# skyplane-project/skyplane

Measured on NVIDIA H100. Metric: chunk-pipeline GB/s (raw input), higher is better.
Workload: dtype u8/u32

## Files before the change

skyplane_b200/csrc/lz4.cuh:

```cuda
#pragma once
#include <stdint.h>

namespace sky {

constexpr uint32_t kBlock = 65536;
#ifndef SKY_LZ4_ENTRIES
#define SKY_LZ4_ENTRIES 4096
#endif
constexpr uint32_t kEntries = SKY_LZ4_ENTRIES;
constexpr uint32_t kTableBytes = kEntries * 4;
constexpr uint32_t kMinMatch = 4;
constexpr uint32_t kMfLimit = 12;
constexpr uint32_t kLastLiterals = 5;
constexpr unsigned kFull = 0xffffffffu;

__device__ __forceinline__ void warp_copy(uint8_t *dst, const uint8_t *src, uint32_t n, unsigned lane) {
    if (n < 64) {
        for (uint32_t base = 0; base < n; base += 32) {
            const uint32_t k = base + lane;
            uint8_t b = 0;
            if (k < n) b = src[k];
            __syncwarp();
            if (k < n) dst[k] = b;
        }
// ... 181 lines not shown
__device__ __forceinline__ void sts16(uint32_t a, uint32_t v) { asm volatile("st.shared.u16 [%0], %1;" ::"r"(a), "h"((uint16_t)v) : "memory"); }

__device__ __forceinline__ void mbar_init(uint64_t *bar, uint32_t count) {
    asm volatile("mbarrier.init.shared::cta.b64 [%0], %1;" ::"r"(smem_u32(bar)), "r"(count) : "memory");
}
__device__ __forceinline__ void mbar_arrive(uint64_t *bar) {
    asm volatile("mbarrier.arrive.shared::cta.b64 _, [%0];" ::"r"(smem_u32(bar)) : "memory");
}
__device__ __forceinline__ void mbar_arrive_expect_tx(uint64_t *bar, uint32_t bytes) {
    asm volatile("mbarrier.arrive.expect_tx.shared::cta.b64 _, [%0], %1;" ::"r"(smem_u32(bar)), "r"(bytes) : "memory");
}
__device__ __forceinline__ bool mbar_try_wait(uint64_t *bar, uint32_t parity) {
    uint32_t ok;
    asm volatile("{\n\t.reg .pred p;\n\tmbarrier.try_wait.parity.shared::cta.b64 p, [%1], %2;\n\tselp.u32 %0, 1, 0, p;\n\t}"
                 : "=r"(ok) : "r"(smem_u32(bar)), "r"(parity) : "memory");
    return ok != 0;
}
__device__ __forceinline__ bool mbar_try_wait_hint(uint64_t *bar, uint32_t parity, uint32_t ns) {
    uint32_t ok;
    asm volatile("{\n\t.reg .pred p;\n\tmbarrier.try_wait.parity.shared::cta.b64 p, [%1], %2, %3;\n\tselp.u32 %0, 1, 0, p;\n\t}"
                 : "=r"(ok) : "r"(smem_u32(bar)), "r"(parity), "r"(ns) : "memory");
    return ok != 0;
}
__device__ __forceinline__ void mbar_wait(uint64_t *bar, uint32_t parity) {
    while (!mbar_try_wait_hint(bar, parity, 20000u)) {}
}
__device__ __forceinline__ void bulk_load(void *smem_dst, const void *gsrc, uint32_t bytes, uint64_t *bar) {
    asm volatile("cp.async.bulk.shared::cluster.global.mbarrier::complete_tx::bytes [%0], [%1], %2, [%3];"
                 ::"r"(smem_u32(smem_dst)), "l"(gsrc), "r"(bytes), "r"(smem_u32(bar)) : "memory");
}

__device__ __forceinline__ uint32_t div255(uint32_t x) { return (x * 0x8081u) >> 23; }
__device__ __forceinline__ uint32_t seq_bytes_fast(uint32_t ll, uint32_t ml) {
    uint32_t s = 1 + ll + (ll >= 15 ? div255(ll - 15) + 1 : 0);
    if (ml) s += 2 + (ml >= 19 ? div255(ml - 19) + 1 : 0);
    return s;
}
__device__ __forceinline__ uint32_t load32s(uint32_t in_s, uint32_t pos) {
    const uint32_t a = in_s + (pos & ~3u);
    return __funnelshift_r(lds32(a), lds32(a + 4), (pos & 3u) * 8u);
}

template <class Load4>
__device__ __forceinline__ uint32_t extend_coop(Load4 load4, uint32_t mpos, uint32_t mcand, uint32_t mlen, uint32_t maxlen, unsigned lane) {
    for (;;) {
        const uint32_t o = mlen + lane * 4;
        uint32_t cnt = 0;
        if (o < maxlen) {
            const uint32_t x = load4(mpos + o) ^ load4(mcand + o);
            cnt = x ? (uint32_t)(__ffs(x) - 1) >> 3 : 4u;
            cnt = min(cnt, maxlen - o);
        }
        const unsigned fullm = __ballot_sync(kFull, cnt == 4);
        if (fullm == kFull) {
            mlen += 128;
            continue;
        }
        const int f = __ffs(~fullm) - 1;
        return mlen + 4 * f + __shfl_sync(kFull, cnt, f);
    }
}
__device__ __forceinline__ uint32_t extend_coop_s(uint32_t in32, uint32_t mpos, uint32_t mcand, uint32_t mlen, uint32_t maxlen,
                                                  unsigned lane) {
    return extend_coop([in32](uint32_t pos) { return load32s(in32, pos); }, mpos, mcand, mlen, maxlen, lane);
}

__device__ __noinline__ uint32_t flush_seqs(uint8_t *__restrict__ out, uint32_t op, const uint8_t *in, uint32_t q0, uint32_t q1,
                                            uint32_t nseq, bool skip_first, unsigned lane) {
    const uint32_t in32 = smem_u32(in);
    const bool act = lane < nseq && !(skip_first && lane == 0);
    const uint32_t ll = q0 & 0xffffu, ml = q0 >> 16, lit = q1 & 0xffffu, off = q1 >> 16;
    const uint32_t mcode = ml - kMinMatch;
    const uint32_t nl = ll >= 15 ? div255(ll - 15) + 1 : 0, nm = mcode >= 15 ? div255(mcode - 15) + 1 : 0;
    const uint32_t sz = act ? 3 + ll + nl + nm : 0;
    uint32_t incl = sz;
#pragma unroll
    for (int d = 1; d < 32; d <<= 1) {
        const uint32_t t = __shfl_up_sync(kFull, incl, d);
        if ((int)lane >= d) incl += t;
    }
    const uint32_t total = __shfl_sync(kFull, incl, 31);
    uint32_t lit_o = 0;
    if (act) {
        uint32_t o = op + incl - sz;
        out[o++] = (uint8_t)(((ll < 15 ? ll : 15) << 4) | (mcode < 15 ? mcode : 15));
        if (nl) {
            for (uint32_t k = 0; k + 1 < nl; k++) out[o + k] = 255;
            out[o + nl - 1] = (uint8_t)(ll - 15 - (nl - 1) * 255);
            o += nl;
        }
        lit_o = o;
        if (ll < kCoopLit) {
            uint32_t k = 0;
            for (; k + 4 <= ll; k += 4) {
                const uint32_t w = load32s(in32, lit + k);
                out[o + k] = (uint8_t)w;
                out[o + k + 1] = (uint8_t)(w >> 8);
                out[o + k + 2] = (uint8_t)(w >> 16);
                out[o + k + 3] = (uint8_t)(w >> 24);
            }
            const uint32_t rem = ll - k;
            if (rem) {
                const uint32_t w = load32s(in32, lit + k);
                out[o + k] = (uint8_t)w;
                if (rem > 1) out[o + k + 1] = (uint8_t)(w >> 8);
                if (rem > 2) out[o + k + 2] = (uint8_t)(w >> 16);
            }
        }
        o += ll;
        out[o] = (uint8_t)off;
        out[o + 1] = (uint8_t)(off >> 8);
        o += 2;
        if (nm) {
            for (uint32_t k = 0; k + 1 < nm; k++) out[o + k] = 255;
            out[o + nm - 1] = (uint8_t)(mcode - 15 - (nm - 1) * 255);
        }
    }
    __syncwarp();
    unsigned big = __ballot_sync(kFull, act && ll >= kCoopLit);
    while (big) {
        const int l = __ffs(big) - 1;
        big &= big - 1;
        warp_copy(out + __shfl_sync(kFull, lit_o, l), in + __shfl_sync(kFull, lit, l), __shfl_sync(kFull, ll, l), lane);
    }
    return op + total;
}

__device__ __forceinline__ uint32_t bfind(uint32_t x) {
    uint32_t r;
    asm("bfind.u32 %0, %1;" : "=r"(r) : "r"(x));
    return r;
}
__device__ __forceinline__ void near_slot(uint32_t &n, uint32_t hf, uint32_t c3, uint32_t c4, uint32_t c8) {
    asm volatile(
        "{\n\t"
        ".reg .pred p, q;\n\t"
        ".reg .b32 t;\n\t"
        "shfl.sync.up.b32 t|p, %1, 8, 0, 0xffffffff;\n\t"
        "setp.eq.and.u32 q, t, %1, p;\n\t"
        "selp.u32 %0, %4, %0, q;\n\t"
        "shfl.sync.up.b32 t|p, %1, 4, 0, 0xffffffff;\n\t"
        "setp.eq.and.u32 q, t, %1, p;\n\t"
        "selp.u32 %0, %3, %0, q;\n\t"
        "shfl.sync.up.b32 t|p, %1, 3, 0, 0xffffffff;\n\t"
        "setp.eq.and.u32 q, t, %1, p;\n\t"
        "selp.u32 %0, %2, %0, q;\n\t"
        "}"
        : "+r"(n)
        : "r"(hf), "r"(c3), "r"(c4), "r"(c8));
}
__device__ __forceinline__ void red_max_s(uint32_t a, uint32_t v) {
    asm volatile("red.shared.max.u32 [%0], %1;" ::"r"(a), "r"(v) : "memory");
}
template <class Turn>
__device__ __forceinline__ uint32_t probe_batch(uint32_t in_s, uint32_t tab_s, uint32_t offs_s, uint32_t masks_s, uint32_t seg_pos,
                                                uint32_t slog, uint32_t batch, uint32_t mflimit, unsigned lane, Turn turn) {
    const uint32_t pstep = 32u << slog;
    uint32_t p = seg_pos + ((batch * 256u + lane) << slog);
    const uint32_t selv = 0x3210u + 0x1111u * (p & 3u), selb = 0x4440u | (p & 3u);
    const uint32_t offs_l = offs_s + (batch * 256u + lane) * 2u;
    const uint32_t c3 = 0x30000u << slog, c4 = 0x40000u << slog, c8 = 0x80000u << slog;
    uint32_t idx[8], mine[8], e[8], near[8], anyhit = 0;
#pragma unroll
    for (int k = 0; k < 8; k++) {
        const uint32_t pc = min(p, mflimit);
        const uint32_t a = in_s + (pc & ~3u);
        const uint32_t w0 = lds32(a), w1 = lds32(a + 4);
        uint32_t hf = __byte_perm(w0, w1, selv) * 2654435761u;
        hf = __byte_perm(w1, 0u, selb) * 0x85EBCA6Bu + hf;
        idx[k] = __umulhi(hf, kEntries) * 4u;
        mine[k] = __byte_perm(p, hf, 0x1065);
        near[k] = 0u;
        near_slot(near[k], hf, c3, c4, c8);
        p += pstep;
    }
    turn();
#pragma unroll
    for (int k = 0; k < 8; k++) {
        e[k] = lds32(tab_s + idx[k]);
        __syncwarp();
        red_max_s(tab_s + idx[k], mine[k]);
        __syncwarp();
    }
#pragma unroll
    for (int k = 0; k < 8; k++) {
        uint32_t d = mine[k] - e[k];
        if (near[k]) d = near[k];
        const uint32_t off = d >> 16;
        const unsigned hits = __ballot_sync(kFull, (d & 0xffffu) == 0u && off != 0u);
        anyhit |= hits;
        if (lane == 0) sts32(masks_s + (batch * 8u + (uint32_t)k) * 4u, hits);
        sts16(offs_l + (uint32_t)k * 64u, off);
    }
    return anyhit;
}

__device__ __forceinline__ SegRec parse_segment(const uint8_t *in, const SegSlot *slot, uint8_t *__restrict__ scr, uint32_t L,
                                                unsigned lane) {
    const uint32_t in32 = smem_u32(in), offs_s = smem_u32(slot->offs);
    const uint32_t seg_pos = slot->seg_pos, slog = slot->slog;
    const uint32_t mflimit = L - kMfLimit, matchlimit = L - kLastLiterals;
    const uint32_t n_real = ((mflimit - seg_pos) >> slog) + 1u;
    const uint32_t mymask = slot->masks[lane] & ~__funnelshift_lc(0u, 0xffffffffu, min(max(n_real, lane * 32u) - lane * 32u, 32u));
    const uint32_t seg_lim = seg_pos + (kSegSlots << slog);
    const uint32_t mlim = min(matchlimit, seg_lim);
    const uint32_t seg_end = seg_lim > mflimit ? L : seg_lim;
    const uint32_t round_up = (1u << slog) - 1u;
    const uint32_t dl = lane < 23 ? lane : lane - 32u;
    const uint32_t jrel = lane < 23 ? lane : 31u - lane;
    const bool fwd_lane = lane < 23;
    uint32_t anchor = seg_pos, cur = seg_pos, nseq = 0, q0 = 0, q1 = 0, mbytes = 0;
    uint32_t first_q0 = 0, first_q1 = 0;
    bool first_pending = true;
    unsigned nz = __ballot_sync(kFull, mymask != 0u);
    uint32_t m = 0, gbase = 0, sbase = 0;
    for (;;) {
        if (m == 0) {
            if (nz == 0) break;
            const int g = __ffs(nz) - 1;
            nz &= nz - 1;
            m = __shfl_sync(kFull, mymask, g);
            sbase = (uint32_t)g * 32u;
            gbase = seg_pos + (sbase << slog);
            m &= __funnelshift_lc(0u, 0xffffffffu, (max(cur, gbase) - gbase + round_up) >> slog);
            if (m == 0) continue;
        }
        const uint32_t bit = bfind(m & (0u - m));
        uint32_t pos = gbase + (bit << slog);
        const uint32_t off = lds16(offs_s + (sbase + bit) * 2u);
        const uint32_t cand = pos - off;
        const uint32_t maxlen = mlim - pos;
        const uint32_t room = min(min(pos - anchor, cand), 8u);
        bool ok = false;
        if (jrel < (fwd_lane ? maxlen : room)) ok = lds8(in32 + pos + dl) == lds8(in32 + cand + dl);
        const unsigned z = ~__ballot_sync(kFull, ok) | 0x00800000u;
        uint32_t mlen = bfind(z & (0u - z));
        if (mlen - kMinMatch >= 23u - kMinMatch) {
            if (mlen < kMinMatch) {
                m &= m - 1;
                continue;
            }
            if (maxlen > 23u) mlen = extend_coop_s(in32, pos, cand, 23u, maxlen, lane);
        }
        const uint32_t back = (uint32_t)__clz(z);
        const uint32_t end = pos + mlen;
        pos -= back;
        mlen += back;
        const uint32_t r0 = (pos - anchor) | (mlen << 16), r1 = anchor | (off << 16);
        if (lane == nseq) {
            q0 = r0;
            q1 = r1;
        }
        anchor = cur = end;
        m &= __funnelshift_lc(0u, 0xffffffffu, (cur - gbase + round_up) >> slog);
        if (++nseq == 32) {
            if (first_pending) {
                first_q0 = __shfl_sync(kFull, q0, 0);
                first_q1 = __shfl_sync(kFull, q1, 0);
            }
            mbytes = flush_seqs(scr, mbytes, in, q0, q1, 32, first_pending, lane);
            first_pending = false;
            nseq = 0;
        }
    }
    if (nseq) {
        if (first_pending) {
            first_q0 = __shfl_sync(kFull, q0, 0);
            first_q1 = __shfl_sync(kFull, q1, 0);
        }
        mbytes = flush_seqs(scr, mbytes, in, q0, q1, nseq, first_pending, lane);
    }
    SegRec r;
    r.seg_pos = seg_pos;
    r.lead_ml = first_q0;
    r.off_t = (first_q1 >> 16) | ((seg_end - anchor) << 16);
    r.mbytes = mbytes;
    return r;
}

}
```

skyplane_b200/csrc/skychunk.cu:

```cuda

#include <cuda_runtime.h>
#include <stdint.h>
#include <stdio.h>
#include <string.h>

#include <algorithm>
#include <memory>
#include <new>
#include <numeric>
#include <string>
#include <utility>
#include <vector>

#include "../../include/skychunk.h"
#include "frame.cuh"
#include "lz4.cuh"
#include "lz4dec.cuh"
#include "lz4hc.cuh"
#include "lz4verify.cuh"
#include "md5.cuh"
#include "secretbox.cuh"

namespace sky {

#ifndef SKY_PARSERS
#define SKY_PARSERS 12
#endif
constexpr int kParsers = SKY_PARSERS;
constexpr int kProbers = 2;
constexpr int kWarps = kProbers + kParsers;
constexpr int kThreads = kWarps * 32;
#ifndef SKY_RING_EXTRA
#define SKY_RING_EXTRA 2
#endif
constexpr int kRing = kParsers + SKY_RING_EXTRA;
constexpr int kMd5WarpsPerCta = 4;
constexpr uint32_t kRingBytes = SKY_MD5_SLOTS * 2048;
constexpr int kCtasPerSm = 2;
constexpr uint64_t kMaxChunkBlocks = 1ull << 21;

struct Ctl {
    uint64_t in_full;
    uint64_t full[kRing], empty[kRing];
    BlockDesc desc[2];
    uint32_t claim;
    volatile uint32_t block_end_seq;
    volatile uint32_t nseg;
    volatile uint32_t seg_hit[4];
    uint32_t raw, last_lits, tail_off;
    uint64_t data;
    uint32_t size;
    PendingChecksum pend;
};
constexpr uint32_t kInOff = 0;
constexpr uint32_t kTabOff = kInOff + kInBytes;
constexpr uint32_t kRingOff = kTabOff + kTableBytes;
constexpr uint32_t kRecOff = kRingOff + kRing * (uint32_t)sizeof(SegSlot);
constexpr uint32_t kPlanOff = kRecOff + kMaxSegs * (uint32_t)sizeof(SegRec);
constexpr uint32_t kCtlOff = kPlanOff + kMaxSegs * (uint32_t)sizeof(SegPlan);
constexpr uint32_t kSmemBytes = (kCtlOff + (uint32_t)sizeof(Ctl) + 127u) & ~127u;
static_assert(kSmemBytes <= 232448 / 2 - 1024, "two CTAs per SM need <= 112.5 KiB each: lower SKY_PARSERS or SKY_LZ4_ENTRIES");
static_assert(kEntries % 128 == 0, "SKY_LZ4_ENTRIES must be a multiple of 128");
static_assert(kMd5WarpsPerCta * kRingBytes <= kInBytes, "the MD5 rings live in the block buffer of a digest CTA");
static_assert(sizeof(SegSlot) % 16 == 0 && sizeof(SegRec) == 16 && sizeof(SegPlan) == 16, "layout");

template <int kId>
__device__ __forceinline__ void bar_arrive() { asm volatile("bar.arrive %0, 64;" ::"n"(kId) : "memory"); }
template <int kId>
__device__ __forceinline__ void bar_wait() { asm volatile("bar.sync %0, 64;" ::"n"(kId) : "memory"); }

template <bool kXxh, bool kBlkChk>
__device__ __forceinline__ void fused_body(const Params &p) {
    extern __shared__ __align__(128) uint8_t smem[];
    const unsigned warp = threadIdx.x >> 5, lane = threadIdx.x & 31;
    uint8_t *in = smem + kInOff;
    uint32_t *tab = reinterpret_cast<uint32_t *>(smem + kTabOff);
    SegSlot *ring = reinterpret_cast<SegSlot *>(smem + kRingOff);
    SegRec *recs = reinterpret_cast<SegRec *>(smem + kRecOff);
    SegPlan *plans = reinterpret_cast<SegPlan *>(smem + kPlanOff);
    Ctl *ctl = reinterpret_cast<Ctl *>(smem + kCtlOff);
    uint32_t smem_s = smem_u32(smem);
    asm volatile("" : "+r"(smem_s));

    const bool do_md5 = (p.flags & SKY_F_MD5) != 0, do_lz4 = (p.flags & SKY_F_LZ4) != 0;
    if (warp == 0 && lane == 0) {
        mbar_init(&ctl->in_full, 1);
        for (int i = 0; i < kRing; i++) {
            mbar_init(&ctl->full[i], 1);
            mbar_init(&ctl->empty[i], 1);
        }
        ctl->claim = 0;
        if constexpr (kBlkChk) ctl->pend.data = nullptr;
        asm volatile("fence.mbarrier_init.release.cluster;" ::: "memory");
    }
    __syncthreads();

    if (do_md5 && blockIdx.x < p.n_md5_ctas) {
        if (warp < kMd5WarpsPerCta) {
            for (uint32_t g = warp * p.n_md5_ctas + blockIdx.x; g < p.n_groups; g += p.n_md5_ctas * kMd5WarpsPerCta) {
                const uint32_t c = p.md5_order[g * 32 + lane];
                const bool active = c != 0xffffffffu;
                const uint8_t *src = nullptr;
                uint64_t len = 0;
                if (active) {
                    src = p.chunks[c].src;
                    len = p.chunks[c].len;
                }
                const uint32_t x = md5_warp<kXxh>(reinterpret_cast<uint32_t *>(in + warp * kRingBytes), src, len, active,
                                                  p.md5_out + (size_t)(active ? c : 0) * 16, lane);
                if constexpr (kXxh) {
                    if (active) p.xxh_out[c] = x;
                }
                __syncwarp();
            }
        }
        if (!do_lz4) return;
        __syncthreads();
    }
    if (!do_lz4) return;

    uint8_t *scratch = p.scratch + (size_t)blockIdx.x * kScratchBytes;
    uint32_t gseq = 0;
    uint32_t batches_done = 0;
    uint32_t my_seq = 0;
    bool have_claim = false;
    uint32_t in_phase = 0;
    constexpr unsigned kSumWarp = kWarps - 1;
    for (uint32_t it = 0;; it++) {
        BlockDesc *dsc = &ctl->desc[it & 1];
        if (warp == 0 && lane == 0) {
            claim_block(p, dsc);
            ctl->block_end_seq = 0xffffffffu;
            ctl->nseg = 0;
        }
        __syncthreads();
        if (!dsc->valid) {
            if constexpr (kBlkChk) {
                if (warp == kSumWarp) run_pending(&ctl->pend, lane);
            }
            break;
        }
        const uint8_t *src = dsc->src;
        const uint32_t L = dsc->L;

        if (warp < kProbers) {
            if (warp == 0) {
                if (lane == 0) load_block(in, src, L, &ctl->in_full);
                uint4 *t4 = reinterpret_cast<uint4 *>(tab);
                const uint4 z = make_uint4(0, 0, 0, 0);
#pragma unroll 4
                for (uint32_t k = lane; k < kEntries / 4; k += 32) t4[k] = z;
                __syncwarp();
            }
            mbar_wait(&ctl->in_full, in_phase);
            in_phase ^= 1;
            uint32_t nseg = 0;
            if (L >= kMfLimit + 1) {
                const uint32_t mflimit = L - kMfLimit;
                uint32_t seg_pos = 0, slog = 0;
                while (seg_pos <= mflimit) {
                    if (nseg >= 2) {
                        const bool h = ctl->seg_hit[(nseg - 2) & 3u] != 0u;
                        slog = h ? 0u : min(slog + 1u, kMaxStepLog);
                    }
                    const uint32_t si = gseq % kRing, ph = (gseq / kRing) & 1u;
                    SegSlot *slot = ring + si;
#pragma unroll 1
                    for (uint32_t b = warp; b < 4; b += kProbers) {
                        const uint32_t slot_s = smem_s + kRingOff + si * (uint32_t)sizeof(SegSlot);
                        const uint32_t hits = probe_batch(smem_s + kInOff, smem_s + kTabOff, slot_s + (uint32_t)offsetof(SegSlot, offs),
                                                          slot_s + (uint32_t)offsetof(SegSlot, masks), seg_pos, slog, b, mflimit, lane, [&]() {
                            if (warp == 0) {
                                if (batches_done) bar_wait<2>();
                                if (b == 0) mbar_wait(&ctl->empty[si], ph ^ 1u);
                            } else {
                                bar_wait<1>();
                            }
                        });
                        batches_done = 1;
                        if (lane == 0) {
                            ctl->seg_hit[nseg & 3u] = (b == 0 ? 0u : ctl->seg_hit[nseg & 3u]) | hits;
                            if (b == 0) {
                                slot->seg_pos = seg_pos;
                                slot->slog = slog;
                                slot->sidx = nseg;
                            }
                        }
                        __syncwarp();
                        if (b == 3 && lane == 0) mbar_arrive(&ctl->full[si]);
                        __threadfence_block();
                        if (warp == 0) bar_arrive<1>(); else bar_arrive<2>();
                    }
                    seg_pos += kSegSlots << slog;
                    gseq++;
                    nseg++;
                }
            }
            if (warp == kProbers - 1 && lane == 0) {
                ctl->nseg = nseg;
                __threadfence_block();
                atomicExch(const_cast<uint32_t *>(&ctl->block_end_seq), gseq);
            }
        } else {
            mbar_wait(&ctl->in_full, in_phase);
            in_phase ^= 1;
            for (;;) {
                if (!have_claim) {
                    uint32_t t = 0;
                    if (lane == 0) t = atomicAdd(&ctl->claim, 1u);
                    my_seq = __shfl_sync(kFull, t, 0);
                    have_claim = true;
                }
                const uint32_t si = my_seq % kRing, ph = (my_seq / kRing) & 1u;
                bool got = true;
                while (!mbar_try_wait_hint(&ctl->full[si], ph, 1000u)) {
                    if (atomicAdd(const_cast<uint32_t *>(&ctl->block_end_seq), 0u) <= my_seq) {
                        got = mbar_try_wait(&ctl->full[si], ph);
                        break;
                    }
                }
                if (!got) break;
                const SegSlot *slot = ring + si;
                const uint32_t sidx = slot->sidx;
                uint8_t *scr = scratch + slot->seg_pos + sidx * kSegPad;
                const SegRec r = parse_segment(in, slot, scr, L, lane);
                __syncwarp();
                if (lane == 0) {
                    mbar_arrive(&ctl->empty[si]);
                    recs[sidx] = r;
                }
                have_claim = false;
                if constexpr (kBlkChk) {
                    if (warp == kSumWarp) run_pending(&ctl->pend, lane);
                }
            }
        }
        __syncthreads();

        const uint32_t nseg = ctl->nseg;
        if (warp == 0) {
            constexpr uint32_t kPlanPerLane = (kMaxSegs + 31) / 32;
            uint32_t csize = 0;
            {
                const uint32_t s0 = lane * kPlanPerLane;
                uint32_t has = 0, val = 0;
                for (uint32_t k = 0; k < kPlanPerLane; k++) {
                    const uint32_t sg = s0 + k;
                    if (sg < nseg) {
                        const SegRec r = recs[sg];
                        const uint32_t t = r.off_t >> 16;
                        if (r.lead_ml >> 16) { has = 1; val = t; } else val += t;
                    }
                }
                uint32_t ihas = has, ival = val;
#pragma unroll
                for (int d = 1; d < 32; d <<= 1) {
                    const uint32_t ph_ = __shfl_up_sync(kFull, ihas, d), pv = __shfl_up_sync(kFull, ival, d);
                    if ((int)lane >= d && !ihas) { ihas = ph_; ival += pv; }
                }
                uint32_t carry = __shfl_up_sync(kFull, ival, 1);
                if (lane == 0) carry = 0;
                const uint32_t carry_end = __shfl_sync(kFull, ival, 31);
                uint32_t fll[kPlanPerLane], fsz[kPlanPerLane], msz[kPlanPerLane], mine_total = 0;
#pragma unroll
                for (uint32_t k = 0; k < kPlanPerLane; k++) {
                    const uint32_t sg = s0 + k;
                    fll[k] = fsz[k] = msz[k] = 0;
                    if (sg < nseg) {
                        const SegRec r = recs[sg];
                        const uint32_t ml = r.lead_ml >> 16, t = r.off_t >> 16;
                        msz[k] = r.mbytes;
                        if (ml) {
                            fll[k] = carry + (r.lead_ml & 0xffffu);
                            fsz[k] = seq_bytes_fast(fll[k], ml);
                            carry = t;
                        } else carry += t;
                        mine_total += fsz[k] + msz[k];
                    }
                }
                uint32_t incl = mine_total;
#pragma unroll
                for (int d = 1; d < 32; d <<= 1) {
                    const uint32_t t = __shfl_up_sync(kFull, incl, d);
                    if ((int)lane >= d) incl += t;
                }
                uint32_t o = incl - mine_total;
                const uint32_t total = __shfl_sync(kFull, incl, 31);
#pragma unroll
                for (uint32_t k = 0; k < kPlanPerLane; k++) {
                    const uint32_t sg = s0 + k;
                    if (sg < nseg) {
                        SegPlan pl;
                        pl.foff = o;
                        pl.moff = o + fsz[k];
                        pl.fll = fll[k];
                        pl.pad = 0;
                        plans[sg] = pl;
                        o += fsz[k] + msz[k];
                    }
                }
                const uint32_t last = nseg == 0 ? L : carry_end;
                if (lane == 0) {
                    ctl->last_lits = last;
                    ctl->tail_off = total;
                }
                csize = total + 1 + last + (last >= 15 ? (last - 15) / 255 + 1 : 0);
            }
            if (lane == 0) {
                const BlockPlace pl = place_block<kBlkChk>(p, *dsc, csize, L);
                ctl->raw = pl.raw;
                ctl->data = pl.data;
                if constexpr (kBlkChk) ctl->size = pl.raw ? L : csize;
            }
        }
        __syncthreads();

        {
            uint8_t *out = dsc->dst + ctl->data;
            if (ctl->raw) {
                copy_block<kWarps, true>(out, src, L, warp, lane);
            } else {
                for (uint32_t s = warp; s < nseg; s += kWarps) {
                    const SegRec r = recs[s];
                    const SegPlan pl = plans[s];
                    const uint32_t ml = r.lead_ml >> 16;
                    if (ml) {
                        const uint32_t lit_start = r.seg_pos + (r.lead_ml & 0xffffu) - pl.fll;
                        emit_seq(out, pl.foff, src, lit_start, pl.fll, ml, r.off_t & 0xffffu, lane);
                    }
                    if (r.mbytes) warp_copy_stream<false>(out + pl.moff, scratch + r.seg_pos + s * kSegPad, r.mbytes, lane);
                }
                if (warp == kWarps - 1) {
                    const uint32_t ll = ctl->last_lits;
                    emit_seq(out, ctl->tail_off, src, L - ll, ll, 0, 0, lane);
                }
            }
            if constexpr (kBlkChk) {
                if (warp == kSumWarp) {
                    run_pending(&ctl->pend, lane);
                    set_pending(&ctl->pend, out, ctl->size, lane);
                }
            }
        }
    }
}

__global__ void __launch_bounds__(kThreads, 2) sky_fused_kernel(const Params p) { fused_body<false, false>(p); }
__global__ void __launch_bounds__(kThreads, 2) sky_fused_xxh_kernel(const Params p) { fused_body<true, false>(p); }
__global__ void __launch_bounds__(kThreads, 2) sky_fused_bc_kernel(const Params p) { fused_body<false, true>(p); }
__global__ void __launch_bounds__(kThreads, 2) sky_fused_xxh_bc_kernel(const Params p) { fused_body<true, true>(p); }

__global__ void sky_checksum_kernel(const ChunkDesc *chunks, const uint32_t *xxh, uint64_t *out_len, uint32_t n) {
    const uint32_t c = blockIdx.x * blockDim.x + threadIdx.x;
    if (c >= n) return;
    finish_frame(chunks[c].dst, out_len + c, xxh[c]);
}


struct DecParams {
    DecChunk *chunks;
    DecBlock *blocks;
    int32_t *status;
    uint32_t *dec_done;
    uint32_t *counter;
    uint32_t *blk_done;
    const uint32_t *md5_order;
    uint8_t *md5_out;
    uint32_t n_chunks;
    uint32_t n_groups;
    uint32_t rows;
};

__global__ void sky_frame_index_kernel(const DecParams p) {
    const uint32_t c = blockIdx.x * blockDim.x + threadIdx.x;
    if (c >= p.n_chunks) return;
    DecChunk cd = p.chunks[c];
    int32_t st = kDecOk;
    frame_index(cd, p.blocks + cd.blk_base, &st);
    p.chunks[c].linked = cd.linked;
    p.chunks[c].checks = cd.checks;
    p.chunks[c].content_xxh = cd.content_xxh;
    p.status[c] = st;
}

struct DecRowGate {
    const uint32_t *flags;
    __device__ __forceinline__ void operator()(uint64_t row, bool wants) const {
        unsigned ns = 128;
        for (;;) {
            const bool ready = !wants || ld_relaxed32(flags + row) != 0;
            if (__all_sync(kFull, ready)) break;
            __nanosleep(ns);
            if (ns < 4096) ns <<= 1;
        }
        asm volatile("fence.acq_rel.gpu;" ::: "memory");
    }
};

__global__ void __launch_bounds__(512, 1) sky_decode_kernel(const DecParams p) {
    extern __shared__ __align__(128) uint8_t smem[];
    const unsigned warp = threadIdx.x >> 5, lane = threadIdx.x & 31;
    if (warp < kMd5WarpsPerCta) {
        const uint32_t md5_slots = gridDim.x * kMd5WarpsPerCta;
        for (uint32_t g = warp * gridDim.x + blockIdx.x; g < p.n_groups; g += md5_slots) {
            const uint32_t c = p.md5_order[g * 32 + lane];
            const bool active = c != 0xffffffffu;
            const uint8_t *src = nullptr;
            uint64_t len = 0;
            DecRowGate gate{nullptr};
            if (active) {
                src = p.chunks[c].out;
                len = p.chunks[c].raw_len;
                gate.flags = p.blk_done + p.chunks[c].blk_base;
            }
            const uint32_t x = md5_warp<true>(reinterpret_cast<uint32_t *>(smem + warp * kRingBytes), src, len, active,
                                              p.md5_out + (size_t)(active ? c : 0) * 16, lane, gate);
            if (active) {
                const int32_t s = settle_status(*reinterpret_cast<volatile int32_t *>(p.status + c));
                if (s != kDecOk) p.status[c] = s;
                else if ((p.chunks[c].checks & kChkContent) && x != p.chunks[c].content_xxh) atomicCAS(p.status + c, kDecOk, kDecChecksum);
            }
            __syncwarp();
        }
    }
    for (uint32_t c, j; claim_row_major(p.counter, p.n_chunks, p.rows, lane, c, j);) {
        const DecChunk cd = p.chunks[c];
        if (j >= cd.nblk) continue;
        int32_t st = *reinterpret_cast<volatile int32_t *>(p.status + c);
        const uint64_t pos = (uint64_t)j * kBlock;
        const uint32_t want = (uint32_t)min((uint64_t)kBlock, cd.raw_len - pos);
        if (cd.linked) {
            if (lane == 0) {
                unsigned ns = 64;
                while (ld_acquire32(p.dec_done + c) < j) {
                    __nanosleep(ns);
                    if (ns < 2048) ns <<= 1;
                }
            }
            __syncwarp();
            st = *reinterpret_cast<volatile int32_t *>(p.status + c);
        }
        if (block_may_run(st, j)) {
            const DecBlock b = p.blocks[cd.blk_base + j];
            const uint32_t sz = b.word & 0x7FFFFFFFu;
            if ((cd.checks & kChkBlock) && xxh32_warp(cd.frame + b.off, sz, lane) != b.chk) {
                st = kDecChecksum;
            } else if (b.word & 0x80000000u) {
                st = sz != want ? kDecLayout : kDecOk;
                if (st == kDecOk) warp_copy(cd.out + pos, cd.frame + b.off, sz, lane);
            } else {
                st = lz4_decode_block(cd.frame + b.off, sz, cd.out, pos, want, cd.linked ? 0 : pos, lane);
            }
            if (st != kDecOk && lane == 0) atomicMin(p.status + c, block_fail(j, st));
        }
        __syncwarp();
        if (lane == 0) {
            __threadfence();
            if (cd.linked) st_release32(p.dec_done + c, j + 1);
            st_release32(p.blk_done + cd.blk_base + j, 1u);
        }
    }
}

__global__ void sky_box_setup_kernel(BoxChunk *bc, uint64_t *blk_base, const ChunkDesc *desc, uint32_t n, uint64_t *out_len,
                                     const uint8_t *frame_slab, uint8_t *box_slab, const uint8_t *nonces, int use_frames) {
    for (uint32_t i = threadIdx.x; i < n; i += blockDim.x) {
        const ChunkDesc d = desc[i];
        BoxChunk b;
        b.box = box_slab + (d.dst - frame_slab) + 64ull * i + 8;
        b.msg = use_frames ? d.dst : d.src;
        b.len = use_frames ? out_len[i] : d.len;
        for (int k = 0; k < 24; k++) b.box[k] = nonces[24ull * i + k];
        bc[i] = b;
        out_len[i] = b.len + kBoxOverhead;
    }
    __syncthreads();
    if (threadIdx.x == 0) {
        uint64_t acc = 0;
        for (uint32_t i = 0; i < n; i++) {
            blk_base[i] = acc;
            acc += box_stream_blocks(bc[i].len);
        }
        blk_base[n] = acc;
    }
}

}

using namespace sky;

template <class H, auto Release>
class Owned {
    H h_ = nullptr;

  public:
    Owned() = default;
// ... 784 lines not shown
    DecodeArrays &d = s.dec;
    uint64_t nblk_total = 0;
    uint32_t rows;
    rc = batch_geometry(n, raw_len, rows, [&](uint32_t i, uint32_t nblk) {
        d.h_chunks[i] = DecChunk{d_frames + frame_off[i], d_out + out_off[i], frame_len[i], raw_len[i], nblk_total, nblk, 0};
        nblk_total += nblk;
    });
    if (rc == SKY_OK) rc = grow_block_table(ctx, st, d.table, nblk_total + 1);
    if (rc != SKY_OK) return rc;
    BatchMeta &m = s.meta;
    CK(ctx, cudaMemcpyAsync(d.d_chunks, d.h_chunks, n * sizeof(DecChunk), cudaMemcpyHostToDevice, st));
    CK(ctx, cudaMemsetAsync(m.counters, 0, 64, st));
    CK(ctx, cudaMemsetAsync(d.d_dec_done, 0, n * sizeof(uint32_t), st));
    CK(ctx, cudaMemsetAsync(d.d_status, 0, n * sizeof(int32_t), st));
    CK(ctx, cudaMemsetAsync(d.table.done, 0, (nblk_total + 1) * sizeof(uint32_t), st));
    const uint32_t ng = fill_md5_order(m.h_order, n, raw_len);
    CK(ctx, cudaMemcpyAsync(m.d_order, m.h_order, ng * 32 * sizeof(uint32_t), cudaMemcpyHostToDevice, st));
    memset(m.md5.h, 0, (size_t)n * 16);
    DecParams p;
    p.chunks = d.d_chunks;
    p.blocks = d.table.blocks;
    p.status = d.d_status;
    p.dec_done = d.d_dec_done;
    p.counter = m.counters;
    p.blk_done = d.table.done;
    p.md5_order = m.d_order;
    p.md5_out = m.md5.d;
    p.n_chunks = n;
    p.n_groups = ng;
    p.rows = rows;
    CK(ctx, cudaEventRecord(s.ev_k0, st));
    sky_frame_index_kernel<<<(n + 127) / 128, 128, 0, st>>>(p);
    CK(ctx, cudaGetLastError());
    sky_decode_kernel<<<ctx->sm_count, 512, kMd5WarpsPerCta * kRingBytes, st>>>(p);
    CK(ctx, cudaGetLastError());
    CK(ctx, cudaEventRecord(s.ev_k1, st));
    ctx->launches += 2;
    CK(ctx, cudaMemcpyAsync(d.h_status, d.d_status, n * sizeof(int32_t), cudaMemcpyDeviceToHost, st));
    return SKY_OK;
}

int sky_decode_device(sky_ctx *ctx, uint32_t n, const void *d_frames, const uint64_t *frame_off, const uint64_t *frame_len,
                      void *d_out, const uint64_t *out_off, const uint64_t *raw_len, void *stream, int32_t *status, uint8_t *md5,
                      float *kernel_ms) {
    if (!ctx || n == 0 || !d_frames || !frame_off || !frame_len || !out_off || !raw_len) return SKY_E_INVALID;
    if (n > ctx->max_chunks) return SKY_E_CAPACITY;
    if (reinterpret_cast<uintptr_t>(d_out) & 15) return SKY_E_INVALID;
    for (uint32_t i = 0; i < n; i++) {
        if (out_off[i] & 15) return SKY_E_INVALID;
        if (raw_len[i] && !d_out) return SKY_E_INVALID;
    }
    CK(ctx, cudaSetDevice(ctx->device));
    Slot &s = ctx->slots[0];
    if (s.ticket.busy) return SKY_E_BUSY;
    cudaStream_t st = stream ? (cudaStream_t)stream : s.stream;
    int rc = launch_decode(ctx, s, st, n, (const uint8_t *)d_frames, frame_off, frame_len, (uint8_t *)d_out, out_off, raw_len);
    if (rc != SKY_OK) return rc;
    CK(ctx, cudaStreamSynchronize(st));
    if (status) memcpy(status, s.dec.h_status, n * sizeof(int32_t));
    if (md5) memcpy(md5, s.meta.md5.h, (size_t)n * 16);
    if (kernel_ms) CK(ctx, cudaEventElapsedTime(kernel_ms, s.ev_k0, s.ev_k1));
    return SKY_OK;
}

static int decode_raw(sky_ctx *ctx, Slot &s, uint32_t n, const void *const *payload, const uint64_t *payload_len, void *const *dst,
                      const uint64_t *raw_len, bool e2ee, int32_t *status, uint8_t *md5, float *kernel_ms) {
    std::vector<uint64_t> off(n), box_off(n), msg_len(payload_len, payload_len + n), md5_len(n);
    uint64_t ip = 0, bp = 0;
    for (uint32_t i = 0; i < n; i++) {
        if (payload_len[i] && !payload[i]) return SKY_E_INVALID;
        if (e2ee && raw_len[i] && !dst[i]) return SKY_E_INVALID;
        if (e2ee) msg_len[i] = payload_len[i] >= (uint64_t)kBoxOverhead ? payload_len[i] - kBoxOverhead : 0;
        md5_len[i] = msg_len[i] == raw_len[i] ? raw_len[i] : 0;
        off[i] = ip;
        box_off[i] = bp;
        ip += round16(e2ee ? msg_len[i] : md5_len[i]);
        bp += round16(payload_len[i]);
    }
    if (ip > ctx->in_cap || (e2ee && bp > ctx->out_cap)) return SKY_E_CAPACITY;
    if (e2ee) {
        const int rc = launch_open(ctx, s, n, payload, payload_len, box_off.data(), s.d_in, off.data(), msg_len.data());
        if (rc != SKY_OK) return rc;
    } else {
        for (uint32_t i = 0; i < n; i++)
            if (md5_len[i]) CK(ctx, cudaMemcpyAsync(s.d_in + off[i], payload[i], md5_len[i], cudaMemcpyHostToDevice, s.stream));
    }
    int rc = launch_batch(ctx, s, s.stream, s.stream, n, s.d_in, off.data(), md5_len.data(), s.d_out, off.data(), SKY_F_MD5);
    if (rc != SKY_OK) return rc;
    CK(ctx, cudaStreamSynchronize(s.stream));
    for (uint32_t i = 0; i < n; i++) {
        int32_t st = msg_len[i] == raw_len[i] ? SKY_D_OK : SKY_D_SIZE;
        if (e2ee && (s.box.h_status[i] != 0 || payload_len[i] < (uint64_t)kBoxOverhead)) st = SKY_D_AUTH;
        if (status) status[i] = st;
        if (md5) {
            if (st == SKY_D_OK) memcpy(md5 + 16ull * i, s.meta.md5.h + 16ull * i, 16);
            else memset(md5 + 16ull * i, 0, 16);
        }
        if (e2ee && st == SKY_D_OK && raw_len[i])
            CK(ctx, cudaMemcpyAsync(dst[i], s.d_in + off[i], raw_len[i], cudaMemcpyDeviceToHost, s.stream));
    }
    if (e2ee) CK(ctx, cudaStreamSynchronize(s.stream));
    if (kernel_ms) CK(ctx, cudaEventElapsedTime(kernel_ms, e2ee ? (cudaEvent_t)s.box.ev_open : (cudaEvent_t)s.ev_k0, s.ev_k1));
    return SKY_OK;
}

int sky_decode(sky_ctx *ctx, uint32_t n, const void *const *frames, const uint64_t *frame_len, void *const *dst,
               const uint64_t *raw_len, uint32_t flags, int32_t *status, uint8_t *md5, float *kernel_ms) {
    if (flags & ~(SKY_F_LZ4 | SKY_F_MD5 | SKY_F_E2EE)) return SKY_E_INVALID;
    const bool e2ee = (flags & SKY_F_E2EE) != 0, raw = (flags & (SKY_F_LZ4 | SKY_F_MD5)) == SKY_F_MD5;
    const bool returns_data = !raw || e2ee;
    if (!ctx || n == 0 || !frames || !frame_len || (returns_data && !dst) || !raw_len) return SKY_E_INVALID;
    if (n > ctx->max_chunks) return SKY_E_CAPACITY;
    Slot &s = ctx->slots[0];
    if (s.ticket.busy) return SKY_E_BUSY;
    if (!s.d_in) return SKY_E_INVALID;
    if (e2ee && !ctx->d_key) return SKY_E_NOKEY;
    CK(ctx, cudaSetDevice(ctx->device));
    if (raw) return decode_raw(ctx, s, n, frames, frame_len, dst, raw_len, e2ee, status, md5, kernel_ms);
    std::vector<uint64_t> f_off(n), o_off(n), f_len(frame_len, frame_len + n);
    uint64_t fp = 0, op = 0;
    for (uint32_t i = 0; i < n; i++) {
        if (!frames[i] || (raw_len[i] && !dst[i])) return SKY_E_INVALID;
        f_off[i] = fp;
        o_off[i] = op;
        fp += round16(frame_len[i]);
        op += round16(raw_len[i]);
    }
    if (fp > ctx->out_cap || op > ctx->in_cap) return SKY_E_CAPACITY;
    if (e2ee) {
        int rc = launch_open(ctx, s, n, frames, frame_len, f_off.data(), s.d_out, f_off.data(), f_len.data());
        if (rc != SKY_OK) return rc;
    } else {
        for (uint32_t i = 0; i < n; i++)
            CK(ctx, cudaMemcpyAsync(s.d_out + f_off[i], frames[i], frame_len[i], cudaMemcpyHostToDevice, s.stream));
    }
    int rc = sky_decode_device(ctx, n, s.d_out, f_off.data(), f_len.data(), s.d_in, o_off.data(), raw_len, s.stream, status, md5, kernel_ms);
    if (rc != SKY_OK) return rc;
    if (e2ee) {
        for (uint32_t i = 0; i < n; i++)
            if (s.box.h_status[i] != 0 || frame_len[i] < (uint64_t)kBoxOverhead) {
                s.dec.h_status[i] = SKY_D_AUTH;
                if (status) status[i] = SKY_D_AUTH;
            }
    }
    for (uint32_t i = 0; i < n; i++)
        if (raw_len[i] && s.dec.h_status[i] == 0)
            CK(ctx, cudaMemcpyAsync(dst[i], s.d_in + o_off[i], raw_len[i], cudaMemcpyDeviceToHost, s.stream));
    CK(ctx, cudaStreamSynchronize(s.stream));
    return SKY_OK;
}

uint64_t sky_launch_count(const sky_ctx *ctx) { return ctx ? ctx->launches : 0; }

}
```

Measured before the change: 155.4.

## Let prober warps start the next block while parser warps emit output

Block claim, async load and hash-table clear move to the top of the loop, so every warp waits on the input mbarrier instead of a full-CTA barrier. After probing, the prober warps skip the plan and write phase and go straight to the next block. Planning and output emission are done by the parser warps alone, synchronised with a named barrier, and nseg is double-buffered per block parity. Optional phase-timer instrumentation is added behind a compile flag. The overlap hides write-out latency behind probing, but emission now has fewer warps and there is a risk of races on shared control state across iterations.

```diff
diff --git a/skyplane_b200/csrc/lz4.cuh b/skyplane_b200/csrc/lz4.cuh
--- a/skyplane_b200/csrc/lz4.cuh
+++ b/skyplane_b200/csrc/lz4.cuh
@@ -357,9 +357,9 @@
 __device__ __forceinline__ void red_max_s(uint32_t a, uint32_t v) {
     asm volatile("red.shared.max.u32 [%0], %1;" ::"r"(a), "r"(v) : "memory");
 }
-template <class Turn>
+template <class Turn, class Pass>
 __device__ __forceinline__ uint32_t probe_batch(uint32_t in_s, uint32_t tab_s, uint32_t offs_s, uint32_t masks_s, uint32_t seg_pos,
-                                                uint32_t slog, uint32_t batch, uint32_t mflimit, unsigned lane, Turn turn) {
+                                                uint32_t slog, uint32_t batch, uint32_t mflimit, unsigned lane, Turn turn, Pass pass) {
     const uint32_t pstep = 32u << slog;
     uint32_t p = seg_pos + ((batch * 256u + lane) << slog);
     const uint32_t selv = 0x3210u + 0x1111u * (p & 3u), selb = 0x4440u | (p & 3u);
@@ -387,6 +387,7 @@
         red_max_s(tab_s + idx[k], mine[k]);
         __syncwarp();
     }
+    pass();
 #pragma unroll
     for (int k = 0; k < 8; k++) {
         uint32_t d = mine[k] - e[k];
diff --git a/skyplane_b200/csrc/skychunk.cu b/skyplane_b200/csrc/skychunk.cu
--- a/skyplane_b200/csrc/skychunk.cu
+++ b/skyplane_b200/csrc/skychunk.cu
@@ -45,7 +45,7 @@
     BlockDesc desc[2];
     uint32_t claim;
     volatile uint32_t block_end_seq;
-    volatile uint32_t nseg;
+    volatile uint32_t nseg[2];
     volatile uint32_t seg_hit[4];
     uint32_t raw, last_lits, tail_off;
     uint64_t data;
@@ -68,6 +68,41 @@
 __device__ __forceinline__ void bar_arrive() { asm volatile("bar.arrive %0, 64;" ::"n"(kId) : "memory"); }
 template <int kId>
 __device__ __forceinline__ void bar_wait() { asm volatile("bar.sync %0, 64;" ::"n"(kId) : "memory"); }
+__device__ __forceinline__ void bar_parsers() { asm volatile("bar.sync 3, %0;" ::"n"(kParsers * 32) : "memory"); }
+
+#ifdef SKY_PHASE_TIMERS
+#define SKY_PT(...) __VA_ARGS__
+enum PhaseSlot : int {
+    kPtBlocks, kPtSegs, kPtBatches,
+    kPtCycles, kPtNs,
+    kPtClaim, kPtClear, kPtLoadWait,
+    kPtProbeA0, kPtToken0, kPtTable0, kPtPhaseC0,
+    kPtProbeA1, kPtToken1, kPtTable1, kPtPhaseC1,
+    kPtProberIdle,
+    kPtParseBusy, kPtParseWait, kPtParseIdle,
+    kPtPlan, kPtOffWait,
+    kPtWriteSpan,
+    kPtWriteBusy,
+    kPtSlots = 32
+};
+constexpr int kPtCtas = 1024;
+__device__ unsigned long long g_phase[kPtCtas][kPtSlots];
+__device__ __forceinline__ uint64_t pt_ns() {
+    uint64_t t;
+    asm volatile("mov.u64 %0, %%globaltimer;" : "=l"(t));
+    return t;
+}
+__device__ __forceinline__ void pt_add(int slot, uint64_t v, unsigned lane) {
+    if (lane == 0 && blockIdx.x < kPtCtas) atomicAdd(&g_phase[blockIdx.x][slot], (unsigned long long)v);
+}
+__device__ __forceinline__ void pt_lap(uint64_t &t, int slot, unsigned lane) {
+    const uint64_t n = clock64();
+    pt_add(slot, n - t, lane);
+    t = n;
+}
+#else
+#define SKY_PT(...)
+#endif
 
 template <bool kXxh, bool kBlkChk>
 __device__ __forceinline__ void fused_body(const Params &p) {
@@ -126,34 +161,44 @@
     bool have_claim = false;
     uint32_t in_phase = 0;
     constexpr unsigned kSumWarp = kWarps - 1;
+    SKY_PT(const uint64_t pt_c0 = clock64(), pt_n0 = pt_ns(); uint64_t pt_t = pt_c0, pt_w = 0;)
     for (uint32_t it = 0;; it++) {
         BlockDesc *dsc = &ctl->desc[it & 1];
-        if (warp == 0 && lane == 0) {
-            claim_block(p, dsc);
-            ctl->block_end_seq = 0xffffffffu;
-            ctl->nseg = 0;
+        if (warp == 0) {
+            SKY_PT(uint64_t pt_cl = clock64();)
+            if (lane == 0) {
+                claim_block(p, dsc);
+                ctl->block_end_seq = 0xffffffffu;
+                if (dsc->valid) load_block(in, dsc->src, dsc->L, &ctl->in_full);
+                else mbar_arrive(&ctl->in_full);
+            }
+            SKY_PT(pt_lap(pt_cl, kPtClaim, lane); pt_t = pt_cl;)
+            uint4 *t4 = reinterpret_cast<uint4 *>(tab);
+            const uint4 z = make_uint4(0, 0, 0, 0);
+#pragma unroll 4
+            for (uint32_t k = lane; k < kEntries / 4; k += 32) t4[k] = z;
+            __syncwarp();
+            SKY_PT(pt_lap(pt_t, kPtClear, lane);)
         }
-        __syncthreads();
+        mbar_wait(&ctl->in_full, in_phase);
+        in_phase ^= 1;
+        SKY_PT(if (warp == 0) pt_lap(pt_t, kPtLoadWait, lane); else pt_t = clock64();)
         if (!dsc->valid) {
             if constexpr (kBlkChk) {
                 if (warp == kSumWarp) run_pending(&ctl->pend, lane);
             }
+            SKY_PT(if (warp == 0) {
+                pt_add(kPtCycles, clock64() - pt_c0, lane);
+                pt_add(kPtNs, pt_ns() - pt_n0, lane);
+            })
             break;
         }
+        SKY_PT(if (warp == 0) pt_add(kPtBlocks, 1, lane);)
         const uint8_t *src = dsc->src;
         const uint32_t L = dsc->L;
 
         if (warp < kProbers) {
-            if (warp == 0) {
-                if (lane == 0) load_block(in, src, L, &ctl->in_full);
-                uint4 *t4 = reinterpret_cast<uint4 *>(tab);
-                const uint4 z = make_uint4(0, 0, 0, 0);
-#pragma unroll 4
-                for (uint32_t k = lane; k < kEntries / 4; k += 32) t4[k] = z;
-                __syncwarp();
-            }
-            mbar_wait(&ctl->in_full, in_phase);
-            in_phase ^= 1;
+            SKY_PT(uint32_t pt_b = (uint32_t)clock64(), pt_a = 0, pt_k = 0, pt_tb = 0, pt_c = 0, pt_x = 0, pt_y = 0, pt_z = 0, pt_e = 0;)
             uint32_t nseg = 0;
             if (L >= kMfLimit + 1) {
                 const uint32_t mflimit = L - kMfLimit;
@@ -170,13 +215,15 @@
                         const uint32_t slot_s = smem_s + kRingOff + si * (uint32_t)sizeof(SegSlot);
                         const uint32_t hits = probe_batch(smem_s + kInOff, smem_s + kTabOff, slot_s + (uint32_t)offsetof(SegSlot, offs),
                                                           slot_s + (uint32_t)offsetof(SegSlot, masks), seg_pos, slog, b, mflimit, lane, [&]() {
+                            SKY_PT(pt_x = (uint32_t)clock64();)
                             if (warp == 0) {
                                 if (batches_done) bar_wait<2>();
                                 if (b == 0) mbar_wait(&ctl->empty[si], ph ^ 1u);
                             } else {
                                 bar_wait<1>();
                             }
-                        });
+                            SKY_PT(pt_y = (uint32_t)clock64();)
+                        }, [&]() { SKY_PT(pt_z = (uint32_t)clock64();) });
                         batches_done = 1;
                         if (lane == 0) {
                             ctl->seg_hit[nseg & 3u] = (b == 0 ? 0u : ctl->seg_hit[nseg & 3u]) | hits;
@@ -190,6 +237,8 @@
                         if (b == 3 && lane == 0) mbar_arrive(&ctl->full[si]);
                         __threadfence_block();
                         if (warp == 0) bar_arrive<1>(); else bar_arrive<2>();
+                        SKY_PT(pt_e = (uint32_t)clock64(); pt_a += pt_x - pt_b; pt_k += pt_y - pt_x; pt_tb += pt_z - pt_y;
+                               pt_c += pt_e - pt_z; pt_b = pt_e;)
                     }
                     seg_pos += kSegSlots << slog;
                     gseq++;
@@ -197,13 +246,14 @@
                 }
             }
             if (warp == kProbers - 1 && lane == 0) {
-                ctl->nseg = nseg;
+                ctl->nseg[it & 1] = nseg;
                 __threadfence_block();
                 atomicExch(const_cast<uint32_t *>(&ctl->block_end_seq), gseq);
             }
+            SKY_PT(pt_add(kPtProbeA0 + 4 * warp, pt_a, lane); pt_add(kPtToken0 + 4 * warp, pt_k, lane);
+                   pt_add(kPtTable0 + 4 * warp, pt_tb, lane); pt_add(kPtPhaseC0 + 4 * warp, pt_c, lane);
+                   pt_add(kPtBatches, nseg * 2u, lane); if (warp == 0) pt_add(kPtSegs, nseg, lane); pt_t = clock64();)
         } else {
-            mbar_wait(&ctl->in_full, in_phase);
-            in_phase ^= 1;
             for (;;) {
                 if (!have_claim) {
                     uint32_t t = 0;
@@ -219,6 +269,7 @@
                         break;
                     }
                 }
+                SKY_PT(pt_lap(pt_t, kPtParseWait, lane);)
                 if (!got) break;
                 const SegSlot *slot = ring + si;
                 const uint32_t sidx = slot->sidx;
@@ -233,12 +284,15 @@
                 if constexpr (kBlkChk) {
                     if (warp == kSumWarp) run_pending(&ctl->pend, lane);
                 }
+                SKY_PT(pt_lap(pt_t, kPtParseBusy, lane);)
             }
         }
         __syncthreads();
-
-        const uint32_t nseg = ctl->nseg;
-        if (warp == 0) {
+        SKY_PT(pt_lap(pt_t, warp < kProbers ? kPtProberIdle : kPtParseIdle, lane);)
+        if (warp < kProbers) continue;
+
+        const uint32_t nseg = ctl->nseg[it & 1];
+        if (warp == kProbers) {
             constexpr uint32_t kPlanPerLane = (kMaxSegs + 31) / 32;
             uint32_t csize = 0;
             {
@@ -306,21 +360,25 @@
                 }
                 csize = total + 1 + last + (last >= 15 ? (last - 15) / 255 + 1 : 0);
             }
+            SKY_PT(pt_lap(pt_t, kPtPlan, lane);)
             if (lane == 0) {
                 const BlockPlace pl = place_block<kBlkChk>(p, *dsc, csize, L);
                 ctl->raw = pl.raw;
                 ctl->data = pl.data;
                 if constexpr (kBlkChk) ctl->size = pl.raw ? L : csize;
             }
+            SKY_PT(__syncwarp(); pt_lap(pt_t, kPtOffWait, lane);)
         }
-        __syncthreads();
+        bar_parsers();
+        SKY_PT(pt_w = clock64();)
 
         {
+            const unsigned pw = warp - kProbers;
             uint8_t *out = dsc->dst + ctl->data;
             if (ctl->raw) {
-                copy_block<kWarps, true>(out, src, L, warp, lane);
+                copy_block<kParsers, true>(out, src, L, pw, lane);
             } else {
-                for (uint32_t s = warp; s < nseg; s += kWarps) {
+                for (uint32_t s = pw; s < nseg; s += kParsers) {
                     const SegRec r = recs[s];
                     const SegPlan pl = plans[s];
                     const uint32_t ml = r.lead_ml >> 16;
@@ -341,7 +399,10 @@
                     set_pending(&ctl->pend, out, ctl->size, lane);
                 }
             }
+            SKY_PT(pt_add(kPtWriteBusy, clock64() - pt_w, lane);)
         }
+        bar_parsers();
+        SKY_PT(if (warp == kProbers) pt_add(kPtWriteSpan, clock64() - pt_w, lane);)
     }
 }
 
@@ -1432,4 +1493,17 @@
 
 uint64_t sky_launch_count(const sky_ctx *ctx) { return ctx ? ctx->launches : 0; }
 
-}
+#ifdef SKY_PHASE_TIMERS
+SKY_API uint32_t sky_phase_timers_reset(void) {
+    void *d = nullptr;
+    if (cudaGetSymbolAddress(&d, sky::g_phase) != cudaSuccess) return 0;
+    return cudaMemset(d, 0, sizeof(sky::g_phase)) == cudaSuccess && cudaDeviceSynchronize() == cudaSuccess ? sky::kPtSlots : 0;
+}
+SKY_API uint32_t sky_phase_timers_read(uint64_t *out, uint32_t max_ctas) {
+    const size_t n = (size_t)std::min<uint32_t>(max_ctas, sky::kPtCtas) * sky::kPtSlots * sizeof(uint64_t);
+    if (cudaDeviceSynchronize() != cudaSuccess || cudaMemcpyFromSymbol(out, sky::g_phase, n) != cudaSuccess) return 0;
+    return sky::kPtSlots;
+}
+#endif
+
+}
```

New measurement: 153.0 (median of 6 runs). 1.6% lower.
